# jimmyshe/liorf

Measured on AMD Instinct MI355X. Metric: LM iterations/sec (64-line scan vs 200k-pt map), higher is better.
Workload: dtype f32; 1 GPU; kitti64: 120000-pt scan vs 200000-pt local surf map, 30 LM iterations per scan (early exit off), one scan per GPU at a time, 8 distinct seeded scans in rotation, map replicated; n_q=120000, n_m=200000, distinct_scans=8, parallelism=scan-per-gpu x1

## Files before the change

include/liorf_s2m_debug.h:

```cpp
#ifndef LIORF_S2M_DEBUG_H
#define LIORF_S2M_DEBUG_H

#include "liorf_s2m.h"

#ifdef __cplusplus
extern "C" {
#endif

int  s2m_debug_device_trig(s2m_handle h, const float* x, size_t n, float* s, float* c, float* a);
int  s2m_debug_deferred(s2m_handle h, int slot);
int  s2m_time_iteration_kernel(s2m_handle h, const float pose[6], int reps, float* ms_per_launch);
int  s2m_time_iterations(s2m_handle h, const float pose[6], int reps, float* ms_per_iter, int cap);

int  s2m_time_loop_launches(s2m_handle h, const float pose[6], int reps, float* us_per_launch);

int  s2m_debug_time_steady(s2m_handle h, const float pose[6], int reps, int solve_prev, float* us_per_launch);

#define S2M_PROF_WORDS 32
int  s2m_debug_wave_profile(s2m_handle h, const float pose[6], int launches, uint64_t* out, size_t cap_waves);

int  s2m_debug_device_hypot(s2m_handle h, const float* x, const float* y, size_t n, float* r);

typedef struct s2m_debug_lm_close_out {
    float   AtA[36], AtB[6];
    int32_t n_sel_last;
    s2m_iter_trace trace;
    float   pose[6];
    float   pose_next[6];
    int32_t iters_run, converged, done, stalled, is_degenerate;
    int32_t n_rows_active;
    float   matP[36];
} s2m_debug_lm_close_out;
int  s2m_debug_lm_close(s2m_handle h, int form, int iter, const double* rows, int n_rows, const float pose0[6],
// ... 100 lines not shown
```

liorf_amd/csrc/s2m_abi.hip:

```cpp
#include <hip/hip_runtime.h>

#include <cfloat>
#include <cmath>
#include <cstdio>
#include <cstdlib>
#include <cstring>
#include <algorithm>
#include <limits>
#include <map>
#include <new>
#include <string>
#include <vector>

#include "s2m_context.hpp"
#include "s2m_kernels.hpp"

using namespace s2m;
using namespace s2m::host;

float s2m::host::stamps_ms(const s2m_context* h, int from, int to)
{
    const unsigned long long a = h->reg.h_stamps[from], b = h->reg.h_stamps[to];
    return (b > a && h->reg.wall_clock_khz > 0) ? (float)((double)(b - a) / (double)h->reg.wall_clock_khz) : 0.0f;
}
// ... 121 lines not shown
inline void launch_certify(s2m_context* h, const LoopShape& sh, int L, int solve_prev, bool fused_loop)
{
    constexpr int NW = kBlock / 64;
    const int fl = solve_prev ? kFlagSolvePrev : 0;
    if (!fused_loop && sh.wpb == NW && h->tune.lean_certify)
        hipLaunchKernelGGL((k_certify_lean<NW, 1, kCertifyLeanWaves>), dim3(sh.nblocks, sh.nslots), dim3(NW * 64), 0, h->stream, sh.tbl, L);
    else if (sh.wpb == kBigWaves) launch_k<false, kBigWaves, kCertifyWavesBig, kCertify, kBigWaves>(h->stream, sh, L, fl);
    else                     launch_k<false, NW, kCertifyWaves, kCertify, NW>(h->stream, sh, L, fl);
}

}

void s2m::host::launch_fused(s2m_context* h, const LoopShape& sh, bool hook, int L, int solve_prev)
{
    constexpr int NW = kBlock / 64;
    const int fl = solve_prev ? kFlagSolvePrev : 0;
    if (sh.wpb == kBigWaves) {
        if (hook) launch_k<true, kBigWaves, 4, kFused, kBigWaves>(h->stream, sh, L, fl);
        else      launch_k<false, kBigWaves, 4, kFused, kBigWaves>(h->stream, sh, L, fl);
    } else if (sh.batch && h->tune.batch_minw == 4 && !hook) {
        launch_k<false, NW, 4, kFused, NW>(h->stream, sh, L, fl);
    } else {
        if (hook) launch_k<true, NW, 2, kFused, NW>(h->stream, sh, L, fl);
        else      launch_k<false, NW, 2, kFused, NW>(h->stream, sh, L, fl);
    }
}

void s2m::host::launch_iteration(s2m_context* h, const LoopShape& sh, int L, int solve_prev, bool fused_loop)
{
    if (!sh.split) { launch_fused(h, sh, false, L, solve_prev); return; }
    if (L == 0) { launch_search(h, sh, 0, true); return; }
    launch_certify(h, sh, L, solve_prev, fused_loop);
    launch_search(h, sh, L, false, sh.late);
    if (h->reg.last_loop.first_split < 0) h->reg.last_loop.first_split = L;
}

void s2m::host::launch_finalize(s2m_context* h, const LoopShape& sh, int L, int mode, bool ends_range)
{
    hipLaunchKernelGGL(k_finalize, dim3(1, sh.nslots), dim3(kFinThreads), 0, h->stream, sh.tbl, L, mode,
                       ends_range ? sh.out : (DevState*)nullptr, ends_range ? sh.stamp : (unsigned long long*)nullptr);
}

void s2m::host::launch_density_wishes(s2m_context* h, const LoopShape& sh)
{
    hipLaunchKernelGGL(k_wave_density, dim3((sh.table_cap + 3) / 4, sh.nslots), dim3(256), 0, h->stream, sh.tbl, h->tune.density_raw);
}
void s2m::host::launch_density_table(s2m_context* h, const LoopShape& sh)
// ... 181 lines not shown
    if (hipGetDeviceCount(&count) != hipSuccess || count <= 0 || prm.device_id < 0 || prm.device_id >= count)
        return S2M_ERR_NO_DEVICE;
    if (hipSetDevice(prm.device_id) != hipSuccess) return S2M_ERR_NO_DEVICE;
    hipDeviceProp_t prop;
    if (hipGetDeviceProperties(&prop, prm.device_id) != hipSuccess) return S2M_ERR_NO_DEVICE;
    if (strncmp(prop.gcnArchName, "gfx950", 6) != 0) return S2M_ERR_NO_DEVICE;

    s2m_context* h = new (std::nothrow) s2m_context();
    if (!h) return S2M_ERR_HIP;
    h->prm = prm; h->device = prm.device_id;
    if (const char* e = getenv("S2M_NO_GRAPH")) h->tune.use_graph = !(e[0] == '1');
    if (const char* e = getenv("S2M_NO_FUSE")) h->tune.fuse_solve = !(e[0] == '1');
    if (const char* e = getenv("S2M_DENSITY_RAW")) h->tune.density_raw = atoi(e);
    if (const char* e = getenv("S2M_BIG_BLOCKS")) h->tune.big_blocks = !(e[0] == '0');
    if (const char* e = getenv("S2M_SEGMENT")) h->tune.seg_iters = atoi(e);
    if (const char* e = getenv("S2M_SPLIT")) h->tune.split_mode = atoi(e);
    if (const char* e = getenv("S2M_LOCKSTEP")) h->tune.lockstep = !(e[0] == '0');
    if (const char* e = getenv("S2M_SPLIT_FROM")) h->tune.split_from = std::max(1, atoi(e));
    if (const char* e = getenv("S2M_SEARCH_GRID")) h->tune.search_grid = std::max(1, atoi(e));
    if (const char* e = getenv("S2M_CLOSE_IN_SEARCH")) h->tune.close_in_search = (e[0] == '1');
    if (const char* e = getenv("S2M_BATCH_MINW")) h->tune.batch_minw = atoi(e);
    if (const char* e = getenv("S2M_BATCH_ENTRIES")) h->tune.batch_entries = atoi(e);
    if (const char* e = getenv("S2M_LEAN")) h->tune.lean_certify = !(e[0] == '0');
    h->tune.fuse_max_blocks = kFuseMaxBlocks;
    if (const char* e = getenv("S2M_FUSE_MAX")) h->tune.fuse_max_blocks = atoi(e);

    auto bail = [&](int code) { s2m_destroy(h); return code; };
    if (prm.stream) { h->stream = static_cast<hipStream_t>(prm.stream); h->own_stream = false; }
    else {
        if (hipStreamCreateWithFlags(&h->stream, hipStreamNonBlocking) != hipSuccess) return bail(S2M_ERR_HIP);
        h->own_stream = true;
    }
    if (hipEventCreate(&h->reg.ev_a) != hipSuccess || hipEventCreate(&h->reg.ev_b) != hipSuccess ||
        hipEventCreate(&h->reg.ev_c) != hipSuccess || hipEventCreate(&h->reg.ev_d) != hipSuccess ||
        hipEventCreate(&h->reg.ev_a2) != hipSuccess || hipEventCreate(&h->reg.ev_b2) != hipSuccess ||
        hipEventCreateWithFlags(&h->reg.ev_up, hipEventDisableTiming) != hipSuccess) return bail(S2M_ERR_HIP);
    static_assert(sizeof(DevState) % 8 == 0, "the trace follows the state block");
    if (hipHostMalloc((void**)&h->reg.h_state, sizeof(DevState) + kSlotStateStride) != hipSuccess) return bail(S2M_ERR_HIP);
    h->reg.h_trace = reinterpret_cast<s2m_iter_trace*>(h->reg.h_state + 2);
    if (hipHostMalloc((void**)&h->reg.h_mm, 64) != hipSuccess) return bail(S2M_ERR_HIP);
    if (hipHostMalloc((void**)&h->reg.h_stamps, sizeof(unsigned long long) * kStampCount) != hipSuccess) return bail(S2M_ERR_HIP);
    memset(h->reg.h_stamps, 0, sizeof(unsigned long long) * kStampCount);
    {
        int khz = 0;
        if (hipDeviceGetAttribute(&khz, hipDeviceAttributeWallClockRate, prm.device_id) != hipSuccess || khz <= 0) { khz = 0; (void)hipGetLastError(); }
        h->reg.wall_clock_khz = khz;
// ... 165 lines not shown
```

liorf_amd/csrc/s2m_abi_debug.hip:

```cpp
#include <hip/hip_runtime.h>

#include <cmath>
#include <cstring>
#include <algorithm>
#include <limits>
#include <vector>

#include "s2m_context.hpp"
#include "s2m_device.hpp"

using namespace s2m;
using namespace s2m::host;

namespace s2m {

__global__ __launch_bounds__(256) void k_debug_sincos(const float* __restrict__ x, int n, float* __restrict__ s, float* __restrict__ c,
                                                      float* __restrict__ a)
{
    const int i = blockIdx.x * blockDim.x + threadIdx.x;
    if (i < n) { s[i] = glibc_sincosf(x[i], 0); c[i] = glibc_sincosf(x[i], 1); if (a) a[i] = glibc_atanf(x[i]); }
}

__global__ __launch_bounds__(256) void k_debug_hypot(const float* __restrict__ x, const float* __restrict__ y, int n, float* __restrict__ r)
{
// ... 312 lines not shown
        S2M_HIP(h, hipMemcpyAsync(qxyz + 2 * n, h->reg.qz.p, sizeof(float) * n, hipMemcpyDeviceToHost, h->stream));
    }
    if (chunk_parts) S2M_HIP(h, hipMemcpyAsync(chunk_parts, h->reg.chunk_parts.p, sizeof(int32_t) * (size_t)n_chunks, hipMemcpyDeviceToHost, h->stream));
    int32_t nw = 0;
    const bool have_table = !h->reg.table_stale;
    if (have_table) S2M_HIP(h, hipMemcpyAsync(&nw, h->reg.n_waves.p, sizeof(nw), hipMemcpyDeviceToHost, h->stream));
    S2M_HIP(h, hipStreamSynchronize(h->stream));
    if (nw < 0 || nw > h->hctx.table_cap) return fail(h, S2M_ERR_HIP, "wave count outside the table");
    if (wave_table && nw > 0) {
        S2M_HIP(h, hipMemcpyAsync(wave_table, h->reg.wave_table.p, sizeof(int2) * (size_t)nw, hipMemcpyDeviceToHost, h->stream));
        S2M_HIP(h, hipStreamSynchronize(h->stream));
    }
    if (n_waves) *n_waves = have_table ? nw : -1;
    return S2M_OK;
}

int s2m_debug_deferred(s2m_handle h, int slot)
{
    if (!h) return S2M_ERR_INVALID_ARG;
    if (slot >= 0) { if (slot >= (int)h->batch.kids.size()) return S2M_ERR_INVALID_ARG; h = h->batch.kids[(size_t)slot]; }
    return h->reg.h_state ? h->reg.h_state[1].deferred_total : 0;
}

static int time_iterations_impl(s2m_handle h, const float pose[6], int reps, float* ms_mean, float* ms_per_iter)
{
    if (!h || !pose || reps < 1) return S2M_ERR_INVALID_ARG;
    if (!h->reg.have_scan || h->reg.n_m == 0 || h->reg.n_q == 0) return fail(h, S2M_ERR_NO_SCAN, "needs a resident scan and map");
    S2M_HIP(h, hipSetDevice(h->device));
    int rc;
    if ((rc = upload_ctx(h))) return rc;
    const int nit = h->prm.max_iter;
    if (h->reg.iter_events.size() < (size_t)(2 * nit)) {
        const size_t old = h->reg.iter_events.size();
        h->reg.iter_events.resize(2 * nit);
        for (size_t k = old; k < h->reg.iter_events.size(); k++) S2M_HIP(h, hipEventCreate(&h->reg.iter_events[k]));
    }
    std::vector<double> per_iter((size_t)nit, 0.0);
    for (int rep = 0; rep < reps; rep++) {
        S2M_HIP(h, hipMemsetAsync(h->reg.cert.p, 0, sizeof(float4) * h->reg.n_q, h->stream));
        S2M_HIP(h, hipMemsetAsync(h->reg.aux.p, 0, sizeof(int4) * h->reg.n_q, h->stream));
        if ((rc = push_state(h, pose))) return rc;
        enqueue_loop(h, shape_of(h), h->reg.iter_events.data());
        h->hctx.density_pending = 0;
        S2M_HIP(h, hipGetLastError());
        S2M_HIP(h, hipStreamSynchronize(h->stream));
        for (int it = 0; it < nit; it++) {
// ... 99 lines not shown
```

liorf_amd/csrc/s2m_context.hpp:

```cpp
#pragma once
#include <hip/hip_runtime.h>

#include <cstddef>
#include <cstdint>
#include <cstdio>
#include <map>
#include <string>
#include <vector>

#include "s2m_types.h"
#include "s2m_host_math.hpp"
#include "s2m_voxel.hpp"
#include "s2m_icp.hpp"
#include "s2m_project.hpp"
#include "s2m_pose_graph.hpp"

namespace s2m {
namespace host __attribute__((visibility("hidden"))) {

struct DevBuf {
    void*  p = nullptr;
    size_t cap = 0;
    DevBuf() = default;
    DevBuf(const DevBuf&) = delete;
// ... 85 lines not shown
        } last;
        int pend_n = 0;
        std::vector<int> live;
        bool seg_pending = false;
        unsigned long long map_epoch = 0;
        unsigned long long adopted_epoch = 0;
    } batch;

    struct Tuning {
        bool use_graph = true;
        bool fuse_solve = true;
        int  fuse_max_blocks = 0;
        int  seg_iters = 8;
        int  split_mode = -1;
        bool tune_env = false;
        bool lean_certify = true;
        int  batch_entries = 1;
        int  batch_minw = 4;
        bool close_in_search = false;
        int  search_grid = 8;
        int  split_from = 8;
        bool lockstep = true;
        bool big_blocks = true;
        int  density_raw = 320;
    } tune;

    struct Voxel {
        DevBuf in, out, frames_xf, scan_ds, map_ds;
        s2m::VoxWorkspace* ws = nullptr;
        size_t scan_ds_n = 0;
        bool have_scan_ds = false;
    } voxel;

    struct ScanContext {
        DevBuf bins, out;
        DevBuf store_desc, store_ring, store_sector, cand;
        DevBuf query, query_part;
        DevBuf many_in, many_qnorm, many_part, many_out;
        unsigned char* h_many = nullptr;
        size_t h_many_cap = 0;
        struct ScPassState { int pass = 0; int last_passes = 0; size_t last_scratch = 0; };
        ScPassState many;
        DevBuf ring_in, ring_cand, ring_dist, ring_out;
        ScPassState ring;
        size_t n = 0, cap = 0, n_search = 0;
        int    counter = 0;
// ... 291 lines not shown
```

liorf_amd/csrc/s2m_prep.hip:

```cpp
#include <hip/hip_runtime.h>

#include <cmath>
#include <cstring>
#include <algorithm>
#include <string>

#include "s2m_context.hpp"
#include "s2m_prep.hpp"

using namespace s2m;
using namespace s2m::host;

namespace {

inline uint32_t host_f2ord(float f) { uint32_t u; memcpy(&u, &f, 4); return (u & 0x80000000u) ? ~u : (u | 0x80000000u); }
inline float host_ord2f(uint32_t o) { uint32_t u = (o & 0x80000000u) ? (o & 0x7fffffffu) : ~o; float f; memcpy(&f, &u, 4); return f; }

int device_exclusive_scan(s2m_context* h, const int32_t* counts, int32_t* out, int n, int total)
{
    const int nb = (n + 1023) / 1024;
    int rc = ensure(h, h->reg.block_sums, sizeof(int32_t) * (size_t)(nb + 1));
    if (rc) return rc;
    int32_t* sums = h->reg.block_sums.as<int32_t>();
    hipLaunchKernelGGL(k_scan_local, dim3(nb), dim3(256), 0, h->stream, counts, out, sums, n);
// ... 112 lines not shown
    h->hctx.map_sorted = h->reg.map_sorted.as<float4>();
    h->hctx.cell_start = h->reg.m_cell_start.as<int32_t>();
    h->ctx_dirty = true;
    S2M_HIP(h, hipEventRecord(h->reg.ev_d, h->stream));
    if ((rc = upload_ctx(h))) return rc;
    S2M_HIP(h, hipStreamSynchronize(h->stream));
    S2M_HIP(h, hipEventElapsedTime(&h->reg.t_set_map_ms, h->reg.ev_c, h->reg.ev_d));
    return S2M_OK;
}

}

int s2m::host::scan_slot_prepare(s2m_context* h, const void* pts, size_t n, size_t stride, bool on_device, PrepSlot* ps)
{
    int rc = check_records(h, pts, n, stride);
    if (rc) return rc;
    memset(ps, 0, sizeof(*ps));
    h->reg.n_q = n; h->reg.have_scan = true;
    h->hctx.n_q = (int32_t)n;
    const int n_chunks = (int)((n + 63) / 64);
    constexpr int NW = kBlock / 64;
    int base_parts = 1;
    while (base_parts < 8 && n_chunks * base_parts * 2 <= 2048) base_parts *= 2;
    h->reg.base_parts = base_parts;
    int nblocks = (n_chunks * base_parts + n_chunks / 2 + NW - 1) / NW;
    nblocks = ((nblocks + kBlocksQuantum - 1) / kBlocksQuantum) * kBlocksQuantum;
    if (nblocks == 0) nblocks = kBlocksQuantum;
    const int table_cap = nblocks * NW;
    const int wpb = (h->tune.big_blocks && n_chunks * base_parts > (kMaxBlocks / 2) * NW) ? kBigWaves : NW;
    nblocks = std::min((table_cap + wpb - 1) / wpb, (wpb == NW && h->batch.parent) ? kMaxBlocks : kMaxBlocks / 2);
    if (h->batch.parent && h->tune.batch_entries > 1) nblocks = std::max((nblocks + h->tune.batch_entries - 1) / h->tune.batch_entries, 1);
    h->hctx.wpb = wpb;
    h->hctx.nblocks = nblocks;
    h->hctx.table_cap = table_cap;
    h->ctx_dirty = true;
    if ((rc = ensure_rows(h, nblocks))) return rc;
    if (n == 0) return S2M_OK;

    const unsigned char* d_pts;
    if (on_device) d_pts = static_cast<const unsigned char*>(pts);
    else {
        if ((rc = stage_host_records(h, h->reg.raw_scan, pts, n * stride))) return rc;
        S2M_HIP(h, hipEventRecord(h->reg.ev_up, h->stream));
        d_pts = h->reg.raw_scan.as<unsigned char>();
    }
    if ((rc = ensure(h, h->reg.qx, sizeof(float) * n))) return rc;
// ... 115 lines not shown
```

liorf_amd/csrc/s2m_register.hpp:

```cpp
#pragma once

constexpr float kCertMargin = 2e-6f;
constexpr float kNbrReach   = 0.15f;
constexpr float kTightBound = 0.62f;
constexpr float kNbrReachCold = 0.10f;
constexpr int   kWalkLanes = 64;
constexpr int   kNbr = kNbrCap;
constexpr float kFragileSlack = 3e-5f;
constexpr float kSlabRound = 1e-6f;
constexpr float kAbsRound = 2.4e-7f;
constexpr int   kTilePad = 32;
constexpr int   kShareMin = 24;
constexpr int   kWalkMax = 384;
constexpr int   kServeLanes = 4;
typedef int v4i __attribute__((ext_vector_type(4)));
typedef float v3f __attribute__((ext_vector_type(3)));

__device__ __forceinline__ uint32_t key_hi(uint64_t k) { return (uint32_t)(k >> 32); }
__device__ __forceinline__ uint32_t key_lo(uint64_t k) { return (uint32_t)k; }
__device__ __forceinline__ void cas_u64(uint64_t& a, uint64_t& b)
{
    const bool c = b < a;
    const uint64_t t = a;
    a = c ? b : a; b = c ? t : b;
// ... 868 lines not shown
        }
    }
}

template <bool HOOK>
__device__ __forceinline__ void linearise_chunk(CtxP cp, const float (&T)[12], const float (&sc6)[6],
                                                int2 chunk, int lane, double (&acc)[kAcc])
{
    const int i = chunk.x + lane;
    if (!(lane < chunk.y && i < cp->n_q)) return;
    const float px = G(cp->qx)[i], py = G(cp->qy)[i], pz = G(cp->qz)[i];
    const v4f pl = G((const v4f*)cp->plane_cache)[i];
    linearise_point<HOOK>(cp, T, sc6, i, px, py, pz, pl, acc);
}

constexpr int kFused = 0, kCertify = 1, kSearch = 2;
constexpr int kCertifyWaves = 4;
constexpr int kCertifyWavesBig = 4;
constexpr int kCertifyLeanWaves = 8;
constexpr int kCertifyLeanEpw = 2;
constexpr int kFlagSolvePrev = 1;
constexpr int kFlagAll = 2;
constexpr int kFlagCloseAfter = 4;
template <int M>
__device__ __forceinline__ double halving_swap_add(double lo, double hi)
{
    typedef unsigned v2u_ __attribute__((ext_vector_type(2)));
    const unsigned long long ul = (unsigned long long)__double_as_longlong(lo), uh = (unsigned long long)__double_as_longlong(hi);
    v2u_ w0, w1;
    if (M == 32) {
        w0 = __builtin_amdgcn_permlane32_swap((unsigned)ul, (unsigned)uh, false, false);
        w1 = __builtin_amdgcn_permlane32_swap((unsigned)(ul >> 32), (unsigned)(uh >> 32), false, false);
    } else {
        w0 = __builtin_amdgcn_permlane16_swap((unsigned)ul, (unsigned)uh, false, false);
        w1 = __builtin_amdgcn_permlane16_swap((unsigned)(ul >> 32), (unsigned)(uh >> 32), false, false);
    }
    const double x = __longlong_as_double((long long)(((unsigned long long)w1.x << 32) | w0.x));
    const double y = __longlong_as_double((long long)(((unsigned long long)w1.y << 32) | w0.y));
    return x + y;
}

__device__ __forceinline__ void wave_reduce16(double (&a)[16], int lane, double* red16 )
{
#pragma unroll
    for (int j = 0; j < 8; j++) a[j] = halving_swap_add<32>(a[j], a[j + 8]);
#pragma unroll
// ... 244 lines not shown
__global__ __launch_bounds__(NW * 64, MINW) void k_register(const SlotTable tbl, int launch, int flags)
{
    static_assert(MODE == kSearch || CNW == NW, "only the search kernel works on another kernel's partition");
    static_assert(CNW % NW == 0, "a search workgroup takes the waves of a row in whole rounds");
    static_assert(!(HOOK && MODE == kCertify), "the observation hook needs the association in line");
    const CtxP cp = ctx_const(tbl.ctx[blockIdx.y]);
    const auto st = G(tbl.st[blockIdx.y]);
    CtxHead ch; StateHead hs;
    load_heads<MODE != kSearch>(cp, st, (MODE != kSearch && (flags & kFlagSolvePrev) != 0) ? (launch - 1) & 1 : launch & 1, ch, hs, launch, flags);
    const int done = hs.done, n_waves = hs.n_waves;
    if (!HOOK && done) return;
    const bool solve_prev = MODE != kSearch && (flags & kFlagSolvePrev) != 0;
    unsigned long long tk_start = 0, clk1 = 0, clk2 = 0;
    unsigned long long lm_stamps[7] = { 0, 0, 0, 0, 0, 0, 0 };
    if (HOOK) tk_start = wall_clock64();

    constexpr bool kHasSearch = MODE != kCertify;
    constexpr int  kTileWaves = kHasSearch ? NW : 1;
    __shared__ v4f     s_pts[kTileWaves][kHasSearch ? kTilePts : 1];
    static_assert(sizeof(v4f) * kTilePts >= sizeof(int32_t) * 18 * 64, "run table must fit the tile area");
    __shared__ double  red[CNW][32];
    __shared__ int2    s_rows[kTileWaves][kHasSearch ? 64 : 1];
    constexpr bool kKeep = kHasSearch && NW == 8 && MINW == 2;
    __shared__ float   s_keep[kKeep ? NW : 1][kKeep ? 7 : 1][kKeep ? 64 : 1];
    __shared__ float   s_lm_out[8];
    __shared__ LmShared s_lm;

    const int tid = threadIdx.x, lane = tid & 63, wave = tid >> 6;
    const int nblocks = ch.nblocks;
    const int nb_act = min((n_waves + CNW - 1) / CNW, nblocks);
    int b = (int)blockIdx.x;
    int wl_cnt = 0, wl_at = (int)blockIdx.x;
    const bool listed = MODE == kSearch && !(flags & kFlagAll);
    if (listed) {
        const auto wlc = G(cp->wl_count);
        wl_cnt = wlc[launch & 1];
        if (b == 0 && tid == 0) { wlc[(launch + 1) & 1] = 0; st->deferred_total += wl_cnt; }
    } else if (MODE == kSearch) {
        if (b == 0 && tid == 0) G(cp->wl_count)[(launch + 1) & 1] = 0;
    }
    for (;;) {
    if (listed) {
        if (wl_at >= wl_cnt) {
            if (!(flags & kFlagCloseAfter)) return;
            break;
        }
        b = __builtin_amdgcn_readfirstlane(G(cp->wl_items)[(size_t)(launch & 1) * (size_t)nblocks + wl_at]);
// ... 115 lines not shown
                if (r != 0 || e != e0) {
                    chunk = make_int2(__builtin_amdgcn_readfirstlane(tb[e].x), __builtin_amdgcn_readfirstlane(tb[e].y));
                    px = 0.0f; py = 0.0f; pz = 0.0f; cert = v4f{ 0, 0, 0, 0 };
                    if (lane < chunk.y && chunk.x + lane < nq) {
                        const int i = chunk.x + lane;
                        px = G(cp->qx)[i]; py = G(cp->qy)[i]; pz = G(cp->qz)[i];
                        cert = G((const v4f*)cp->cert)[i];
                    }
                }
                associate_chunk<HOOK, (MINW > 2), !(NW == 8 && MINW == 4)>(cp, g, map, cell_start, T, gatef, ablate, chunk, lane, s_pts[wave], s_rows[wave],
                                      nullptr, px, py, pz, cert, prof);
            }
            if (HOOK) clk1 = wall_clock64();
#pragma unroll
            for (int k = 0; k < kAcc; k++) acc[k] = 0.0;
            for (int e = e0; e < n_waves; e += estride)
                linearise_chunk<HOOK>(cp, T, sc6, make_int2(tb[e].x, tb[e].y), lane, acc);
            wave_reduce_acc(acc, lane, red[w]);
        }
        if (HOOK) clk2 = wall_clock64();
    } else {
    const bool single = e0 + estride >= n_waves;
    if (__builtin_expect(single, 1)) {
        if (e0 < n_waves) {
            float sx, sy, sz, eps;
            const bool need = lane_needs(T, px, py, pz, cert, valid0, ablate, sx, sy, sz, eps);
            bool quick = false;
            if (!HOOK && __ballot(need) != 0ull) {
                bool okl = true, flip = false;
                const int nfr = min(max(frag.aux.z, 0), kNbr);
                Top6k t;
#pragma unroll
                for (int k = 0; k < 6; k++) t.key[k] = kKeyInf;
                if (need) {
                    okl = frag.on && (frag.aux.y & 12) == 12 && (frag.aux.y & 3) != 0;
#pragma unroll
                    for (int k = 0; k < 6; k++) {
                        float d2;
                        const uint64_t key = make_key(frag.fr[k], sx, sy, sz, d2);
                        t.key[k] = (okl && k < nfr) ? key : kKeyInf;
                    }
                    sort6k(t);
                    const float r = __int_as_float(frag.aux.w) - eps;
                    const float d2_5 = __uint_as_float(key_hi(t.key[4]));
                    okl = okl && key_hi(t.key[4]) < 0x7f800000u && ((double)d2_5 < cp->gate_sq) && (sqrtf(d2_5) + kCertMargin < r);
#pragma unroll
// ... 32 lines not shown
                            const float rr_ = pa * mx[j][0] + pb * mx[j][1] + pc * mx[j][2] + pd;
                            if ((double)fabsf(rr_) > cp->plane_tol) planeValid = false;
                        }
                        pl_new = v4f{ planeValid ? pa : NAN, pb, pc, pd };
                    }
                }
                if (flip) {
                    const int i = chunk.x + lane;
                    G((v4f*)cp->plane_alt)[i] = plane0;
#pragma unroll
                    for (int k = 0; k < 5; k++) G(cp->npos_alt)[(size_t)k * nq + i] = frag.opos[k];
                    G((v4f*)cp->plane_cache)[i] = pl_new;
#pragma unroll
                    for (int k = 0; k < 5; k++) G(cp->npos)[(size_t)k * nq + i] = (int)key_lo(t.key[k]);
                    plane0 = pl_new;
                    const v4f cnew = { cert.x, cert.y, cert.z, 0.0f };
                    G((v4f*)cp->cert)[i] = cnew;
                    const v4i anew = { frag.aux.x, (frag.aux.y & ~3) | ((pl_new.x == pl_new.x) ? 1 : 2) | 16, frag.aux.z, frag.aux.w };
                    G((v4i*)cp->aux)[i] = anew;
                }
            }
            if (MODE == kCertify) {
                defer = __ballot(need) != 0ull && !quick;
            } else if (HOOK || __builtin_expect(__ballot(need) != 0ull && !quick, 0)) {
                float* lkeep = kKeep ? &s_keep[kKeep ? wave : 0][0][0] : nullptr;
                if (kKeep) {
                    lkeep[0 * 64 + lane] = px; lkeep[1 * 64 + lane] = py; lkeep[2 * 64 + lane] = pz;
                    lkeep[3 * 64 + lane] = plane0.x; lkeep[4 * 64 + lane] = plane0.y; lkeep[5 * 64 + lane] = plane0.z; lkeep[6 * 64 + lane] = plane0.w;
                }
                associate_chunk<HOOK, (MINW > 2), !(NW == 8 && MINW == 4)>(cp, g, map, cell_start, T, gatef, ablate, chunk, lane, s_pts[wave], s_rows[wave],
                                      lkeep, px, py, pz, cert, prof);
                asm volatile("" ::: "memory");
                if (kKeep) {
                    wave_lds_sync();
                    px = lkeep[0 * 64 + lane]; py = lkeep[1 * 64 + lane]; pz = lkeep[2 * 64 + lane];
                    plane0 = v4f{ lkeep[3 * 64 + lane], lkeep[4 * 64 + lane], lkeep[5 * 64 + lane], lkeep[6 * 64 + lane] };
                } else if (valid0) {
                    const int i = chunk.x + lane;
                    px = G(cp->qx)[i]; py = G(cp->qy)[i]; pz = G(cp->qz)[i];
                    plane0 = G((const v4f*)cp->plane_cache)[i];
                }
            }
            if (HOOK) clk1 = wall_clock64();
#pragma unroll
            for (int k = 0; k < kAcc; k++) acc[k] = 0.0;
            if (valid0 && !defer) linearise_point<HOOK>(cp, T, sc6, chunk.x + lane, px, py, pz, plane0, acc);
        } else {
#pragma unroll
            for (int k = 0; k < kAcc; k++) acc[k] = 0.0;
        }
    } else {
    bool any_need = HOOK;
    if (!HOOK) {
        for (int e = e0; e < n_waves; e += estride) {
            const int2 en = make_int2(__builtin_amdgcn_readfirstlane(tb[e].x), __builtin_amdgcn_readfirstlane(tb[e].y));
            const int i = en.x + lane;
            bool need = false;
            if (lane < en.y && i < nq) {
                const float qx = G(cp->qx)[i], qy = G(cp->qy)[i], qz = G(cp->qz)[i];
                const v4f ce = G((const v4f*)cp->cert)[i];
                float sx, sy, sz, eps;
                need = lane_needs(T, qx, qy, qz, ce, true, ablate, sx, sy, sz, eps);
            }
            any_need = any_need || (__ballot(need) != 0ull);
        }
    }
    if (MODE == kCertify) defer = any_need;
    else {
    if (__builtin_expect(any_need, 0))
    for (int e = e0; e < n_waves; e += estride) {
        if (e != e0) {
            chunk = make_int2(__builtin_amdgcn_readfirstlane(tb[e].x), __builtin_amdgcn_readfirstlane(tb[e].y));
// ... 76 lines not shown
```

liorf_amd/csrc/s2m_types.h:

```cpp
#pragma once
#include <stddef.h>
#include <stdint.h>
#include <hip/hip_runtime.h>
#include "../../include/liorf_s2m.h"
#include "../../include/liorf_s2m_debug.h"

namespace s2m {

constexpr int kBlock = 512;
constexpr int kAcc = 28;
constexpr int kFinThreads = 1024;
constexpr int kMaxIter = 64;
constexpr int kProfWords = 32;
constexpr int kBlocksQuantum = 8;
constexpr int kNbrCap = 6;
constexpr int kMaxBlocks = 512;
constexpr int kBigWaves = 16;

struct GridDesc {
    float ox, oy, oz;
    float inv_e;
    float e;
    int   nx, ny, nz;
    int   ncells;
};

struct alignas(64) DevState {
    int32_t done;
    int32_t n_waves;
    int32_t isDegenerate;
    int32_t T_valid;
    float pose2[2][6];
    float T[12];
    float sc[6];
    float pose[6];
    float matP[36];
    float AtA[36];
    float AtB[6];
    int32_t converged;
    int32_t iters_run;
    int32_t n_sel_last;
    int32_t stalled;
    int32_t deferred_total;
};
static_assert(offsetof(DevState, done) == 0 && offsetof(DevState, pose2) == 16 && offsetof(DevState, T) == 64 &&
              offsetof(DevState, sc) == 112 && sizeof(DevState) % 64 == 0, "DevState: the prologue's fields fill the first line");
constexpr size_t kSlotStateStride = sizeof(DevState) + sizeof(s2m_iter_trace) * kMaxIter;
static_assert(kSlotStateStride % 64 == 0, "a batch's state blocks all start on a 64-byte line");

struct alignas(64) DevCtx {
    int32_t nblocks;
    int32_t n_q;
    const int2* wave_table;
    double* partials;
    const float* qx; const float* qy; const float* qz;
    float4*  cert;
    float4*  plane_cache;
    GridDesc g;
    const float4* map_sorted;
    const int32_t* cell_start;
    float  gate_f;
    int32_t ablate;
    int4*    aux;
    float4*  front;
    int32_t* npos;
    float4*  plane_alt;
// ... 59 lines not shown
```

liorf_amd/s2m.py:

```python
from __future__ import annotations

import ctypes as C
import importlib.util
import os
import sys

import numpy as np

_HERE = os.path.dirname(os.path.abspath(__file__))
LIB_PATH = os.environ.get("S2M_LIB") or os.path.join(_HERE, "libliorf_s2m.so")

S2M_OK = 0
S2M_ERR_CAPACITY = -5
S2M_ERR_BUSY = -6
S2M_ERR_FORMAT, S2M_ERR_CHECKSUM, S2M_ERR_IO = -7, -8, -9
ERRORS = {-1: "S2M_ERR_INVALID_ARG", -2: "S2M_ERR_NO_DEVICE", -3: "S2M_ERR_HIP", -4: "S2M_ERR_NO_SCAN",
          -5: "S2M_ERR_CAPACITY", -6: "S2M_ERR_BUSY", -7: "S2M_ERR_FORMAT", -8: "S2M_ERR_CHECKSUM", -9: "S2M_ERR_IO"}

ABI_SYMBOLS = [
    "s2m_version", "s2m_default_params", "s2m_create", "s2m_destroy", "s2m_last_error", "s2m_set_params", "s2m_get_params",
    "s2m_set_map", "s2m_set_map_device", "s2m_set_scan", "s2m_set_scan_device",
    "s2m_optimize", "s2m_optimize_resident", "s2m_optimize_launch", "s2m_optimize_collect",
    "s2m_optimize_batch", "s2m_batch_set_scan", "s2m_batch_set_scans", "s2m_slot_set_scan", "s2m_slot_optimize_launch", "s2m_slot_optimize_collect", "s2m_optimize_batch_launch", "s2m_optimize_batch_collect", "s2m_batch_get_trace",
    "s2m_get_trace", "s2m_surf_optimization", "s2m_normal_eq", "s2m_last_timing", "s2m_debug_deferred",
    "s2m_time_iteration_kernel", "s2m_time_iterations", "s2m_make_scancontext", "s2m_debug_wave_profile", "s2m_debug_time_steady", "s2m_time_loop_launches",
    "s2m_debug_scan_prep",
    "s2m_voxel_downsample", "s2m_voxel_downsample_device", "s2m_downsample_scan", "s2m_extract_cloud",
    "s2m_transform_cloud",
    "s2m_icp_default_params", "s2m_icp_align", "s2m_icp_align_guess", "s2m_debug_device_trig", "s2m_debug_device_hypot",
    "s2m_debug_lm_close", "s2m_debug_lm_close_check_args", "s2m_debug_lm_rows", "s2m_debug_lm_rows_check_args",
    "s2m_sc_reset", "s2m_sc_size", "s2m_sc_add_scan", "s2m_sc_add_descriptor", "s2m_sc_detect_loop", "s2m_sc_distance",
    "s2m_sc_query_default_params", "s2m_sc_query_check_args", "s2m_sc_query_key", "s2m_sc_query_descriptor", "s2m_sc_query_scan", "s2m_sc_query_projected",
    "s2m_sc_query_many_default_params", "s2m_sc_query_many_check_args", "s2m_sc_query_keys", "s2m_sc_query_descriptors", "s2m_sc_get_descriptors",
    "s2m_debug_sc_query_many_pass", "s2m_debug_sc_query_many_shape", "s2m_debug_sc_query_many_last",
    "s2m_sc_ring_default_params", "s2m_sc_ring_check_args", "s2m_sc_ring_neighbours_keys", "s2m_sc_ring_neighbours_descriptors",
    "s2m_sc_query_keys_ring", "s2m_sc_query_descriptors_ring", "s2m_debug_sc_ring_pass", "s2m_debug_sc_ring_shape", "s2m_debug_sc_ring_last",
    "s2m_kf_default_params", "s2m_kf_reset", "s2m_kf_size", "s2m_kf_add", "s2m_kf_set_poses", "s2m_extract_surrounding",
    "s2m_extract_surrounding_at",
    "s2m_loop_default_params", "s2m_loop_near_keyframes", "s2m_loop_align", "s2m_loop_closure_rs",
    "s2m_loop_align_launch", "s2m_loop_closure_rs_launch", "s2m_loop_poll", "s2m_loop_collect",
    "s2m_loop_verify_check_args", "s2m_loop_verify_launch", "s2m_loop_verify_poll", "s2m_loop_verify_collect", "s2m_loop_verify",
    "s2m_loop_verify_many_check_args", "s2m_loop_verify_many", "s2m_debug_icp_align_pairs_device",
    "s2m_debug_loop_verify_many_pass", "s2m_debug_loop_verify_many_last", "s2m_debug_loop_verify_many_plan", "s2m_debug_batch_last",
    "s2m_reloc_default_params", "s2m_relocalize_check_args", "s2m_relocalize_scan", "s2m_debug_icp_align_guess_many_device",
    "s2m_debug_icp_nearest", "s2m_debug_icp_time_nearest", "s2m_debug_icp_align_device", "s2m_debug_icp_align_many_device",
    "s2m_debug_icp_tuning", "s2m_debug_icp_grid_check_args", "s2m_debug_icp_grid",
    "s2m_gmap_default_params", "s2m_global_map", "s2m_kf_map_cloud",
# ... 266 lines not shown
    L.s2m_destroy.argtypes = [vp]
    L.s2m_set_params.argtypes = [vp, C.POINTER(Params)]
    L.s2m_get_params.argtypes = [vp, C.POINTER(Params)]
    for n in ("s2m_set_map", "s2m_set_map_device", "s2m_set_scan", "s2m_set_scan_device"):
        getattr(L, n).argtypes = [vp, vp, C.c_size_t, C.c_size_t]
    L.s2m_optimize.argtypes = [vp, vp, C.c_size_t, C.c_size_t, fp, C.POINTER(ImuInit), C.POINTER(Result)]
    L.s2m_optimize_resident.argtypes = [vp, fp, C.POINTER(ImuInit), C.POINTER(Result)]
    L.s2m_optimize_launch.argtypes = [vp, fp]
    L.s2m_optimize_collect.argtypes = [vp, fp, C.POINTER(ImuInit), C.POINTER(Result)]
    L.s2m_get_trace.argtypes = [vp, C.POINTER(IterTrace), C.c_int]
    L.s2m_optimize_batch.argtypes = [vp, C.c_int, C.POINTER(vp), C.POINTER(C.c_size_t), C.c_size_t, fp, C.POINTER(ImuInit), C.POINTER(Result)]
    L.s2m_batch_set_scan.argtypes = [vp, C.c_int, vp, C.c_size_t, C.c_size_t, C.c_int]
    L.s2m_slot_set_scan.argtypes = [vp, C.c_int, vp, C.c_size_t, C.c_size_t, C.c_int]
    L.s2m_slot_optimize_launch.argtypes = [vp, C.c_int, fp]
    L.s2m_slot_optimize_collect.argtypes = [vp, C.c_int, fp, C.POINTER(ImuInit), C.POINTER(Result)]
    L.s2m_batch_set_scans.argtypes = [vp, C.c_int, C.POINTER(C.c_void_p), C.POINTER(C.c_size_t), C.c_size_t, C.c_int]
    L.s2m_optimize_batch_launch.argtypes = [vp, C.c_int, fp]
    L.s2m_optimize_batch_collect.argtypes = [vp, C.c_int, fp, C.POINTER(ImuInit), C.POINTER(Result)]
    L.s2m_batch_get_trace.argtypes = [vp, C.c_int, C.POINTER(IterTrace), C.c_int]
    L.s2m_surf_optimization.argtypes = [vp, fp, C.POINTER(C.c_int32), fp, C.POINTER(C.c_uint8), fp]
    L.s2m_normal_eq.argtypes = [vp, fp, fp, fp, C.POINTER(C.c_int32)]
    L.s2m_last_timing.argtypes = [vp, fp, fp, fp]
    L.s2m_debug_deferred.argtypes = [vp, C.c_int]
    L.s2m_time_iteration_kernel.argtypes = [vp, fp, C.c_int, fp]
    L.s2m_time_iterations.argtypes = [vp, fp, C.c_int, fp, C.c_int]
    L.s2m_debug_wave_profile.argtypes = [vp, fp, C.c_int, C.POINTER(C.c_uint64), C.c_size_t]
    L.s2m_debug_time_steady.argtypes = [vp, fp, C.c_int, C.c_int, fp]
    L.s2m_time_loop_launches.argtypes = [vp, fp, C.c_int, fp]
    L.s2m_debug_scan_prep.argtypes = [vp, C.c_int32, fp, C.POINTER(C.c_int32), fp, C.POINTER(C.c_int32), C.POINTER(C.c_int32),
                                      C.POINTER(C.c_int32), C.POINTER(C.c_int32)]
    L.s2m_make_scancontext.argtypes = [vp, vp, C.c_size_t, C.c_size_t, C.POINTER(C.c_double), C.POINTER(C.c_double)]
    szp = C.POINTER(C.c_size_t)
    for n in ("s2m_voxel_downsample", "s2m_voxel_downsample_device"):
        getattr(L, n).argtypes = [vp, vp, C.c_size_t, C.c_size_t, C.c_float, vp, C.c_size_t, C.c_size_t, szp]
    L.s2m_downsample_scan.argtypes = [vp, vp, C.c_size_t, C.c_size_t, C.c_int, C.c_float, vp, C.c_size_t, C.c_size_t, szp]
    L.s2m_extract_cloud.argtypes = [vp, C.c_int, C.POINTER(vp), szp, C.c_size_t, C.c_int, fp, C.c_float,
                                    vp, C.c_size_t, C.c_size_t, szp]
    L.s2m_transform_cloud.argtypes = [vp, vp, C.c_size_t, C.c_size_t, fp, vp, C.c_size_t]
    dp, i32p = C.POINTER(C.c_double), C.POINTER(C.c_int32)
    L.s2m_debug_device_trig.argtypes = [vp, fp, C.c_size_t, fp, fp, fp]
    L.s2m_debug_device_hypot.argtypes = [vp, fp, fp, C.c_size_t, fp]
    L.s2m_debug_lm_close.argtypes = [vp, C.c_int, C.c_int, dp, C.c_int, fp, C.c_int, fp, C.POINTER(LmCloseOut)]
    L.s2m_debug_lm_close_check_args.argtypes = [C.c_int, C.c_int, C.c_int, dp, C.c_int, fp, fp, C.POINTER(LmCloseOut)]
    L.s2m_debug_lm_rows.argtypes = [vp, fp, C.c_int, dp, C.c_int, C.POINTER(LmRowsOut), i32p]
    L.s2m_debug_lm_rows_check_args.argtypes = [fp, C.c_int, C.c_int, C.c_int, dp, C.c_int, C.POINTER(LmRowsOut)]
    L.s2m_icp_default_params.argtypes = [C.POINTER(IcpParams)]
# ... 1813 lines not shown
```

Measured before the change: 56140 LM iterations/s.

## Pool idle waves to split neighbour-search chunks of busy waves within a block

Adds an opt-in pooling mode, set by an environment variable, to the fused single-pass kernel. Waves whose points need no neighbour search post their state to shared memory and take a slice of a busy wave's chunk for the association search, so search work is spread across the whole block instead of serialising on a few waves. It also adds a base_parts override, a pool_parts counter in device state, and a debug accessor. The fused variant is restructured even when pooling is off, and shared memory grows (11 keep rows instead of 7, plus a post array). That could lower occupancy, and the pooled path adds block-wide barriers.

```diff
diff --git a/include/liorf_s2m_debug.h b/include/liorf_s2m_debug.h
--- a/include/liorf_s2m_debug.h
+++ b/include/liorf_s2m_debug.h
@@ -9,6 +9,7 @@
 
 int  s2m_debug_device_trig(s2m_handle h, const float* x, size_t n, float* s, float* c, float* a);
 int  s2m_debug_deferred(s2m_handle h, int slot);
+int  s2m_debug_pool_parts(s2m_handle h, int32_t* npos, float* plane, int32_t* state);
 int  s2m_time_iteration_kernel(s2m_handle h, const float pose[6], int reps, float* ms_per_launch);
 int  s2m_time_iterations(s2m_handle h, const float pose[6], int reps, float* ms_per_iter, int cap);
 
diff --git a/liorf_amd/csrc/s2m_abi.hip b/liorf_amd/csrc/s2m_abi.hip
--- a/liorf_amd/csrc/s2m_abi.hip
+++ b/liorf_amd/csrc/s2m_abi.hip
@@ -167,7 +167,7 @@
         launch_k<false, NW, 4, kFused, NW>(h->stream, sh, L, fl);
     } else {
         if (hook) launch_k<true, NW, 2, kFused, NW>(h->stream, sh, L, fl);
-        else      launch_k<false, NW, 2, kFused, NW>(h->stream, sh, L, fl);
+        else      launch_k<false, NW, 2, kFused, NW>(h->stream, sh, L, fl | (h->tune.pool ? kFlagPool : 0));
     }
 }
 
@@ -395,6 +395,8 @@
     if (const char* e = getenv("S2M_BATCH_MINW")) h->tune.batch_minw = atoi(e);
     if (const char* e = getenv("S2M_BATCH_ENTRIES")) h->tune.batch_entries = atoi(e);
     if (const char* e = getenv("S2M_LEAN")) h->tune.lean_certify = !(e[0] == '0');
+    if (const char* e = getenv("S2M_POOL")) h->tune.pool = !(e[0] == '0');
+    if (const char* e = getenv("S2M_BASE_PARTS")) h->tune.base_parts = atoi(e);
     h->tune.fuse_max_blocks = kFuseMaxBlocks;
     if (const char* e = getenv("S2M_FUSE_MAX")) h->tune.fuse_max_blocks = atoi(e);
 
diff --git a/liorf_amd/csrc/s2m_abi_debug.hip b/liorf_amd/csrc/s2m_abi_debug.hip
--- a/liorf_amd/csrc/s2m_abi_debug.hip
+++ b/liorf_amd/csrc/s2m_abi_debug.hip
@@ -358,6 +358,31 @@
     return h->reg.h_state ? h->reg.h_state[1].deferred_total : 0;
 }
 
+int s2m_debug_pool_parts(s2m_handle h, int32_t* npos, float* plane, int32_t* state)
+{
+    if (!h) return S2M_ERR_INVALID_ARG;
+    if (h->reg.pending != Reg::kNone) return fail(h, S2M_ERR_INVALID_ARG, "an optimize launch is pending: collect it first");
+    if (npos || plane || state) {
+        if (!h->reg.have_scan) return fail(h, S2M_ERR_NO_SCAN, "s2m_set_scan has not been called");
+        const size_t n = h->reg.n_q;
+        S2M_HIP(h, hipSetDevice(h->device));
+        if (npos && n) S2M_HIP(h, hipMemcpyAsync(npos, h->reg.npos.p, sizeof(int32_t) * 5 * n, hipMemcpyDeviceToHost, h->stream));
+        if (plane && n) S2M_HIP(h, hipMemcpyAsync(plane, h->reg.plane_cache.p, sizeof(float) * 4 * n, hipMemcpyDeviceToHost, h->stream));
+        std::vector<int4> aux(state ? n : 0);
+        if (state && n) S2M_HIP(h, hipMemcpyAsync(aux.data(), h->reg.aux.p, sizeof(int4) * n, hipMemcpyDeviceToHost, h->stream));
+        std::vector<float4> ms(npos ? h->reg.n_m : 0);
+        if (!ms.empty()) S2M_HIP(h, hipMemcpyAsync(ms.data(), h->reg.map_sorted.p, sizeof(float4) * ms.size(), hipMemcpyDeviceToHost, h->stream));
+        S2M_HIP(h, hipStreamSynchronize(h->stream));
+        for (size_t i = 0; i < aux.size(); i++) state[i] = aux[i].y;
+        for (size_t i = 0; npos && i < 5 * n; i++) {
+            int32_t orig = -1;
+            if (npos[i] >= 0 && (size_t)npos[i] < ms.size()) memcpy(&orig, &ms[(size_t)npos[i]].w, sizeof(orig));
+            npos[i] = orig;
+        }
+    }
+    return h->reg.h_state ? h->reg.h_state[1].pool_parts : 0;
+}
+
 static int time_iterations_impl(s2m_handle h, const float pose[6], int reps, float* ms_mean, float* ms_per_iter)
 {
     if (!h || !pose || reps < 1) return S2M_ERR_INVALID_ARG;
diff --git a/liorf_amd/csrc/s2m_context.hpp b/liorf_amd/csrc/s2m_context.hpp
--- a/liorf_amd/csrc/s2m_context.hpp
+++ b/liorf_amd/csrc/s2m_context.hpp
@@ -131,6 +131,8 @@
         int  split_from = 8;
         bool lockstep = true;
         bool big_blocks = true;
+        bool pool = false;
+        int  base_parts = 0;
         int  density_raw = 320;
     } tune;
 
diff --git a/liorf_amd/csrc/s2m_prep.hip b/liorf_amd/csrc/s2m_prep.hip
--- a/liorf_amd/csrc/s2m_prep.hip
+++ b/liorf_amd/csrc/s2m_prep.hip
@@ -158,6 +158,7 @@
     constexpr int NW = kBlock / 64;
     int base_parts = 1;
     while (base_parts < 8 && n_chunks * base_parts * 2 <= 2048) base_parts *= 2;
+    if (h->tune.base_parts == 1 || h->tune.base_parts == 2 || h->tune.base_parts == 4 || h->tune.base_parts == 8) base_parts = h->tune.base_parts;
     h->reg.base_parts = base_parts;
     int nblocks = (n_chunks * base_parts + n_chunks / 2 + NW - 1) / NW;
     nblocks = ((nblocks + kBlocksQuantum - 1) / kBlocksQuantum) * kBlocksQuantum;
diff --git a/liorf_amd/csrc/s2m_register.hpp b/liorf_amd/csrc/s2m_register.hpp
--- a/liorf_amd/csrc/s2m_register.hpp
+++ b/liorf_amd/csrc/s2m_register.hpp
@@ -914,6 +914,8 @@
 constexpr int kFlagSolvePrev = 1;
 constexpr int kFlagAll = 2;
 constexpr int kFlagCloseAfter = 4;
+constexpr int kFlagPool = 8;
+constexpr int kPoolMinLanes = 8;
 template <int M>
 __device__ __forceinline__ double halving_swap_add(double lo, double hi)
 {
@@ -1204,7 +1206,9 @@
     __shared__ double  red[CNW][32];
     __shared__ int2    s_rows[kTileWaves][kHasSearch ? 64 : 1];
     constexpr bool kKeep = kHasSearch && NW == 8 && MINW == 2;
-    __shared__ float   s_keep[kKeep ? NW : 1][kKeep ? 7 : 1][kKeep ? 64 : 1];
+    constexpr bool kPool = kKeep && !HOOK && MODE == kFused;
+    __shared__ float   s_keep[kKeep ? NW : 1][kKeep ? (kPool ? 11 : 7) : 1][kKeep ? 64 : 1];
+    __shared__ int     s_post[kPool ? 3 : 1][kPool ? NW : 1];
     __shared__ float   s_lm_out[8];
     __shared__ LmShared s_lm;
 
@@ -1366,6 +1370,8 @@
     } else {
     const bool single = e0 + estride >= n_waves;
     if (__builtin_expect(single, 1)) {
+        bool go = false;
+        int n_need = 0;
         if (e0 < n_waves) {
             float sx, sy, sz, eps;
             const bool need = lane_needs(T, px, py, pz, cert, valid0, ablate, sx, sy, sz, eps);
@@ -1444,7 +1450,10 @@
             }
             if (MODE == kCertify) {
                 defer = __ballot(need) != 0ull && !quick;
-            } else if (HOOK || __builtin_expect(__ballot(need) != 0ull && !quick, 0)) {
+            } else if (kPool) {
+                go = __ballot(need) != 0ull && !quick;
+                n_need = go ? __popcll(__ballot(need)) : 0;
+            } else if (HOOK ||__builtin_expect(__ballot(need) != 0ull && !quick, 0)) {
                 float* lkeep = kKeep ? &s_keep[kKeep ? wave : 0][0][0] : nullptr;
                 if (kKeep) {
                     lkeep[0 * 64 + lane] = px; lkeep[1 * 64 + lane] = py; lkeep[2 * 64 + lane] = pz;
@@ -1463,13 +1472,88 @@
                     plane0 = G((const v4f*)cp->plane_cache)[i];
                 }
             }
+            if (!kPool) {
             if (HOOK) clk1 = wall_clock64();
 #pragma unroll
             for (int k = 0; k < kAcc; k++) acc[k] = 0.0;
             if (valid0 && !defer) linearise_point<HOOK>(cp, T, sc6, chunk.x + lane, px, py, pz, plane0, acc);
-        } else {
+            }
+        } else if (!kPool) {
 #pragma unroll
             for (int k = 0; k < kAcc; k++) acc[k] = 0.0;
+        }
+        if (kPool) {
+            const bool pool = (flags & kFlagPool) != 0 && n_waves <= estride;
+            float* lk = &s_keep[kPool ? wave : 0][0][0];
+            int2 sub = go ? chunk : make_int2(0, 0);
+            float qx = px, qy = py, qz = pz;
+            v4f qcert = cert;
+            if (go) {
+                lk[0 * 64 + lane] = px; lk[1 * 64 + lane] = py; lk[2 * 64 + lane] = pz;
+                lk[3 * 64 + lane] = plane0.x; lk[4 * 64 + lane] = plane0.y; lk[5 * 64 + lane] = plane0.z; lk[6 * 64 + lane] = plane0.w;
+                if (pool) { lk[7 * 64 + lane] = cert.x; lk[8 * 64 + lane] = cert.y; lk[9 * 64 + lane] = cert.z; lk[10 * 64 + lane] = cert.w; }
+            }
+            bool any = go;
+            if (pool) {
+                if (lane == 0) { s_post[0][kPool ? wave : 0] = n_need; s_post[kPool ? 1 : 0][kPool ? wave : 0] = chunk.x; s_post[kPool ? 2 : 0][kPool ? wave : 0] = chunk.y; }
+                __syncthreads();
+                int nd[NW], orv = 0;
+#pragma unroll
+                for (int w = 0; w < NW; w++) { nd[w] = __builtin_amdgcn_readfirstlane(s_post[0][kPool ? w : 0]); orv |= nd[w]; }
+                any = orv != 0;
+                if (__builtin_expect(any, 0)) {
+                    const int wv = __builtin_amdgcn_readfirstlane(wave);
+                    int n_search = 0, idle_at = 0;
+#pragma unroll
+                    for (int w = 0; w < NW; w++) { n_search += nd[w] != 0 ? 1 : 0; idle_at += (nd[w] == 0 && w < wv) ? 1 : 0; }
+                    const int n_idle = NW - n_search;
+                    const int trg = idle_at % n_search, part = go ? 0 : idle_at / n_search + 1;
+                    int ow = wv, ox = 0, ocnt = 0, ok = 1, handed = 0;
+#pragma unroll
+                    for (int w = 0; w < NW; w++) {
+                        if (nd[w] != 0) {
+                            int r = 0;
+#pragma unroll
+                            for (int v = 0; v < NW; v++) r += (nd[v] > nd[w] || (nd[v] == nd[w] && v < w)) ? 1 : 0;
+                            const int hlp = n_idle > r ? (n_idle - r - 1) / n_search + 1 : 0;
+                            int k = hlp >= 7 ? 8 : (hlp >= 3 ? 4 : (hlp >= 1 ? 2 : 1));
+                            const int cw = __builtin_amdgcn_readfirstlane(s_post[kPool ? 2 : 0][kPool ? w : 0]);
+                            while (k > 1 && cw / k < kPoolMinLanes) k >>= 1;
+                            handed += k - 1;
+                            if (go ? (w == wv) : (r == trg)) { ow = w; ok = k; ocnt = cw; ox = __builtin_amdgcn_readfirstlane(s_post[kPool ? 1 : 0][kPool ? w : 0]); }
+                        }
+                    }
+                    int off = 0;
+                    sub = make_int2(0, 0);
+                    if (part < ok) {
+                        off = (part * ocnt) / ok;
+                        sub = make_int2(ox + off, ((part + 1) * ocnt) / ok - off);
+                    }
+                    if (!go) {
+                        lk[0 * 64 + lane] = px; lk[1 * 64 + lane] = py; lk[2 * 64 + lane] = pz;
+                        lk[3 * 64 + lane] = plane0.x; lk[4 * 64 + lane] = plane0.y; lk[5 * 64 + lane] = plane0.z; lk[6 * 64 + lane] = plane0.w;
+                        lk = &s_keep[kPool ? ow : 0][0][off];
+                        qx = 0.0f; qy = 0.0f; qz = 0.0f; qcert = v4f{ 0.0f, 0.0f, 0.0f, 0.0f };
+                        if (lane < sub.y) {
+                            qx = lk[0 * 64 + lane]; qy = lk[1 * 64 + lane]; qz = lk[2 * 64 + lane];
+                            qcert = v4f{ lk[(kPool ? 7 : 0) * 64 + lane], lk[(kPool ? 8 : 0) * 64 + lane], lk[(kPool ? 9 : 0) * 64 + lane], lk[(kPool ? 10 : 0) * 64 + lane] };
+                        }
+                    }
+                    if (wv == 0 && lane == 0 && handed > 0) atomicAdd(&tbl.st[blockIdx.y]->pool_parts, handed);
+                }
+            }
+            if (__builtin_expect(any, 0)) {
+                associate_chunk<HOOK, (MINW > 2), !(NW == 8 && MINW == 4)>(cp, g, map, cell_start, T, gatef, ablate, sub, lane, s_pts[wave], s_rows[wave],
+                                      lk, qx, qy, qz, qcert, prof);
+                asm volatile("" ::: "memory");
+                if (pool) __syncthreads(); else wave_lds_sync();
+                const float* own = &s_keep[kPool ? wave : 0][0][0];
+                px = own[0 * 64 + lane]; py = own[1 * 64 + lane]; pz = own[2 * 64 + lane];
+                plane0 = v4f{ own[3 * 64 + lane], own[4 * 64 + lane], own[5 * 64 + lane], own[6 * 64 + lane] };
+            }
+#pragma unroll
+            for (int k = 0; k < kAcc; k++) acc[k] = 0.0;
+            if (valid0) linearise_point<HOOK>(cp, T, sc6, chunk.x + lane, px, py, pz, plane0, acc);
         }
     } else {
     bool any_need = HOOK;
diff --git a/liorf_amd/csrc/s2m_types.h b/liorf_amd/csrc/s2m_types.h
--- a/liorf_amd/csrc/s2m_types.h
+++ b/liorf_amd/csrc/s2m_types.h
@@ -42,6 +42,7 @@
     int32_t n_sel_last;
     int32_t stalled;
     int32_t deferred_total;
+    int32_t pool_parts;
 };
 static_assert(offsetof(DevState, done) == 0 && offsetof(DevState, pose2) == 16 && offsetof(DevState, T) == 64 &&
               offsetof(DevState, sc) == 112 && sizeof(DevState) % 64 == 0, "DevState: the prologue's fields fill the first line");
diff --git a/liorf_amd/s2m.py b/liorf_amd/s2m.py
--- a/liorf_amd/s2m.py
+++ b/liorf_amd/s2m.py
@@ -22,7 +22,7 @@
     "s2m_set_map", "s2m_set_map_device", "s2m_set_scan", "s2m_set_scan_device",
     "s2m_optimize", "s2m_optimize_resident", "s2m_optimize_launch", "s2m_optimize_collect",
     "s2m_optimize_batch", "s2m_batch_set_scan", "s2m_batch_set_scans", "s2m_slot_set_scan", "s2m_slot_optimize_launch", "s2m_slot_optimize_collect", "s2m_optimize_batch_launch", "s2m_optimize_batch_collect", "s2m_batch_get_trace",
-    "s2m_get_trace", "s2m_surf_optimization", "s2m_normal_eq", "s2m_last_timing", "s2m_debug_deferred",
+    "s2m_get_trace", "s2m_surf_optimization", "s2m_normal_eq", "s2m_last_timing", "s2m_debug_deferred", "s2m_debug_pool_parts",
     "s2m_time_iteration_kernel", "s2m_time_iterations", "s2m_make_scancontext", "s2m_debug_wave_profile", "s2m_debug_time_steady", "s2m_time_loop_launches",
     "s2m_debug_scan_prep",
     "s2m_voxel_downsample", "s2m_voxel_downsample_device", "s2m_downsample_scan", "s2m_extract_cloud",
@@ -335,6 +335,7 @@
     L.s2m_normal_eq.argtypes = [vp, fp, fp, fp, C.POINTER(C.c_int32)]
     L.s2m_last_timing.argtypes = [vp, fp, fp, fp]
     L.s2m_debug_deferred.argtypes = [vp, C.c_int]
+    L.s2m_debug_pool_parts.argtypes = [vp, C.POINTER(C.c_int32), fp, C.POINTER(C.c_int32)]
     L.s2m_time_iteration_kernel.argtypes = [vp, fp, C.c_int, fp]
     L.s2m_time_iterations.argtypes = [vp, fp, C.c_int, fp, C.c_int]
     L.s2m_debug_wave_profile.argtypes = [vp, fp, C.c_int, C.POINTER(C.c_uint64), C.c_size_t]
```

After: 55410 LM iterations/s. -1.3%, worse.
